# kakaobrain/hqtransformer

Hardware: AMD Instinct MI355X
Metric: images/sec (256x256 class-cond sampling) (higher is better)
Workload: dtype bf16

## Files before the change

### hqtransformer_amd/csrc/engine.hip

```cpp
#include "../../include/hqt.h"
#include "kernels.h"
#include "fast_kernels.h"
#include "split_kernels.h"
#include "persist.h"

#include <algorithm>
#include <cmath>
#include <cstdarg>
#include <cstdio>
#include <cstring>
#include <map>
#include <memory>
#include <mutex>
#include <string>
#include <vector>

static thread_local std::string g_err;
static int fail(int code, const char* fmt, ...) {
    char buf[1024];
    va_list ap;
    va_start(ap, fmt);
    vsnprintf(buf, sizeof(buf), fmt, ap);
    va_end(ap);
    g_err = buf;
// ... 84 lines not shown
    std::map<std::string, Tensor> w;
    std::vector<void*> owned;
    size_t workspace_bytes = 0;
    int64_t params[3] = {0, 0, 0};
    std::vector<BlockW> body, depth;
    Lin head_top, head_bot;
    int Tmax = 0;
    int max_prefix = 0;
    static constexpr int BODY_BUFS = 10;
    size_t body_bytes[BODY_BUFS] = {};
    int depth_rows = 0;
    int score_chunk = 0;
    int depth_cap() const { return std::max(cfg.max_batch, score_chunk); }
    static constexpr int DEPTH_BUFS = 4;
    size_t depth_bytes[DEPTH_BUFS] = {};
    float *x = nullptr, *xd = nullptr, *logits = nullptr;
    void *hbuf = nullptr, *qbuf = nullptr, *abuf = nullptr, *mbuf = nullptr;
    void *kcache = nullptr, *vcache = nullptr, *dk = nullptr, *dv = nullptr;
    bf16_t *xpk = nullptr, *xdpk = nullptr;
    float *parts = nullptr, *partsd = nullptr;
    int nparts = 0, npartsd = 0;
    float* fold_tmp = nullptr;
    bool tile_gemm = true;
    float* splitk = nullptr;
    size_t splitk_elems = 0;
    struct { const float* slabs; int S; int rows; const float* bias; } pend = {nullptr, 0, 0, nullptr};
    StepState* state = nullptr;
    RowKey* rows = nullptr;
    static constexpr int ROWS_RING = 4;
    RowKey* rows_pinned[ROWS_RING] = {nullptr, nullptr, nullptr, nullptr};
    hipEvent_t rows_ev[ROWS_RING] = {nullptr, nullptr, nullptr, nullptr};
    bool rows_busy[ROWS_RING] = {false, false, false, false};
    int rows_next = 0;
    RowSampler* row_set = nullptr;
    GuidePair* guide = nullptr;
    size_t guide_room() const { return (size_t)std::max(1, cfg.max_batch / 2); }
    unsigned char* keep_mask = nullptr;
    int* group_of_row = nullptr;
    int* row_pos = nullptr;
    struct Staged {
        std::vector<hqt_row_sampler> row_set;
        float* logprob = nullptr;
        std::vector<hqt_guide_pair> guide;
        std::vector<uint8_t> keep;
        int keep_B = 0, keep_n = 0;
        const int64_t* keep_codes[3] = {nullptr, nullptr, nullptr};
// ... 199 lines not shown
        }
    }
    if (c.s1_use_mid_block) {
        add(1, "encoder.mid.block_1", block_in, block_in, res);
        if (c.s1_use_attn) add(2, "encoder.mid.attn_1", block_in, block_in, res);
        add(1, "encoder.mid.block_2", block_in, block_in, res);
    }
    add(7, "encoder", block_in, c.s1_z_channels, res);
}

extern "C" int hqt_abi_version(void) { return HQT_ABI_VERSION; }
extern "C" const char* hqt_last_error(void) { return g_err.c_str(); }

static int alloc_workspace(hqt_handle* hp);

extern "C" int hqt_create(const hqt_config* cfg, int device, hqt_handle** out) {
    if (!cfg || !out) return fail(HQT_ERR_INVALID, "null argument");
    if (cfg->abi_version != HQT_ABI_VERSION) return fail(HQT_ERR_INVALID, "abi_version %d != %d", cfg->abi_version, HQT_ABI_VERSION);
    if (cfg->max_batch < 1) return fail(HQT_ERR_INVALID, "max_batch must be >= 1");
    DeviceGuard dg(device);
    if (!dg.ok) return fail(HQT_ERR_HIP, "hipSetDevice(%d) failed", device);
    std::unique_ptr<hqt_handle> h(new hqt_handle());
    h->tile_gemm = getenv("HQT_NO_TILE_GEMM") == nullptr;
    { const char* e = getenv("HQT_PERSIST"); h->persist_enabled = !(e && atoi(e) == 0); }
    h->single_key = getenv("HQT_NO_SINGLE_KEY") == nullptr;
    h->split_kslices = getenv("HQT_SPLIT_KSLICES_OFF") == nullptr;
    h->cfg = *cfg;
    h->layouts = (cfg->ar_layouts & HQT_LAYOUT_ALL) ? (cfg->ar_layouts & HQT_LAYOUT_ALL) : HQT_LAYOUT_ALL;
    h->device = device;
    const hqt_config& c = h->cfg;
    if (c.has_stage2) {
        if (c.embed_dim % c.n_heads || c.embed_dim % 16) return fail(HQT_ERR_INVALID, "embed_dim must be a multiple of n_heads and 16");
        const int hs = c.embed_dim / c.n_heads;
        if (hs % 8 || hs > 256 || (hs & (hs - 1))) return fail(HQT_ERR_INVALID, "head_dim %d unsupported (power of two in [8, 256])", hs);
        if (c.vocab_top != c.vocab_bot) return fail(HQT_ERR_INVALID, "vocab_top != vocab_bot");
        const bool bidir = c.depth_decoding == HQT_DEPTH_BIDIRECTIONAL;
        if (c.depth_decoding < 0 || c.depth_decoding > HQT_DEPTH_BIDIRECTIONAL || (c.depth_decoding && !bidir && c.code_levels != 3) || (bidir && c.code_levels == 3))
            return fail(HQT_ERR_INVALID, "depth_decoding %d: 0 'parallel-add', 1 'parallel', 2 'parallel-reduce', 3 'top2mid2bot' (three code levels only), "
                        "4 'bidirectional' (two code levels only)", c.depth_decoding);
        if (bidir && c.cond_type == HQT_COND_TEXT)
            return fail(HQT_ERR_INVALID, "depth_decoding 4 'bidirectional' with text conditioning is not built");
        if (c.vocab_top > HQT_MAX_V || c.vocab_top % 4) return fail(HQT_ERR_INVALID, "vocab size %d unsupported", c.vocab_top);
        if (c.cond_type == HQT_COND_CLASS && c.n_classes < 1) return fail(HQT_ERR_INVALID, "n_classes");
        if (c.max_steps < 1 || c.max_steps > c.ctx_len_img) return fail(HQT_ERR_INVALID, "max_steps must be in [1, ctx_len_img]");
    }
    if (c.has_stage1) {
// ... 600 lines not shown
    g.tune = h->policy;
    if (g.alpha == 0.0f) g.alpha = 1.0f;
    if (g.lda == 0) g.lda = l.K;
    if (split_planes) { g.Bw = l.w16h; g.Bw_lo = l.w16l; g.Bw_frag16 = l.wfrag16; g.Bw_up16 = l.wup16; }
}

struct SlotName {
    char s[64];
    SlotName(const char* tag, int rows) {
        static const bool by_rows = getenv("HQT_TIMING_BY_ROWS") != nullptr;
        snprintf(s, sizeof s, by_rows ? "%s@%d" : "%s", tag, rows);
    }
};

static int ar_linear(hqt_handle* h, const Mode& md, GemmArgs g, const Lin& l, int a_dt, int c_dt, hipStream_t st,
                     const char* tag, bool defer_residual = false, int* resid_nparts = nullptr) {
    lin_args(h, g, l, false);
    g.k_quarters = 1;
    const SlotName slot(tag, g.M);
    Timed t(h, slot.s, st);
    if (md.fast) {
        if (resid_nparts) *resid_nparts = g.N / 32;
        if ((g.ln_parts ? l.wpk_ln : l.wpk) && h->tile_gemm && tile_gemm_ok(g, a_dt, c_dt)) {
            const TilePlan tp = tile_gemm_plan(g);
            if (tp.geom >= 0 && (size_t)tp.S * 32 * g.a_packed_mb * g.N <= h->splitk_elems) {
                if (g.ln_parts) g.bias = l.bias_ln;
                HIPCHK(launch_tile_gemm(g, g.ln_parts ? l.wpk_ln : l.wpk, a_dt, c_dt, tp, h->splitk, st));
                if (tp.S > 1) {
                    count_variant(h, "variant:tile_gemm_%dx%d_splitk%d:%s", tp.bm, tp.bn, tp.S, slot.s);
                    t.next(SlotName("gemm_combine", g.M).s);
                    HIPCHK(launch_resid_combine(g, h->splitk, tp.S, st));
                } else count_variant(h, "variant:tile_gemm_%dx%d%s:%s", tp.bm, tp.bn, g.ln_parts ? "_dln" : "", slot.s);
                if (resid_nparts) *resid_nparts = tp.S > 1 ? 1 : g.N / tp.bn;
                return HQT_OK;
            }
        }
        if (g.ln_parts) {
            if (!l.wpk_ln || !stream_gemm_ok(g, a_dt, c_dt)) return fail(HQT_ERR_STATE, "deferred-LayerNorm GEMM without folded weights (%s)", tag);
            g.bias = l.bias_ln;
            HIPCHK(launch_stream_gemm(g, l.wpk_ln, a_dt, c_dt, 1, nullptr, st));
            count_variant(h, "variant:stream_gemm_dln:%s", tag);
            return HQT_OK;
        }
        if (l.wpk && stream_gemm_ok(g, a_dt, c_dt)) {
            int S = (defer_residual && g.store != STORE_RESID) ? stream_gemm_splitk(g) : 1;
            if ((size_t)S * 32 * g.a_packed_mb * g.N > h->splitk_elems) S = 1;
            HIPCHK(launch_stream_gemm(g, l.wpk, a_dt, c_dt, S, h->splitk, st));
            count_variant(h, "variant:stream_gemm:%s", tag);
            if (S > 1) h->pend = {h->splitk, S, 32 * g.a_packed_mb, l.b32};
            return HQT_OK;
        }
        g.Bw = l.w16;
        if (mfma_gemm_ok(g, a_dt, DT_BF16, c_dt)) {
            HIPCHK(launch_mfma_gemm(g, a_dt, DT_BF16, c_dt, st));
            count_variant(h, "variant:mfma_gemm:%s", tag);
// ... 1784 lines not shown
```

### hqtransformer_amd/csrc/fast_kernels.h

```cpp
#pragma once
#include "common.h"
#include "kernels.h"

hipError_t launch_f32_to_bf16(const float* src, bf16_t* dst, size_t n, hipStream_t st);
hipError_t launch_repack_conv(const float* src, float* dst, int O, int I, int taps, hipStream_t st, int Ipad = 0);

bool stream_gemm_supported(int N, int K);
hipError_t launch_pack_stream_weights(const float* w32, bf16_t* packed, int N, int K, hipStream_t st);
hipError_t launch_fold_layernorm(const float* w32, const float* gamma, const float* beta, const float* bias, float* wfold_tmp,
                                 bf16_t* packed, float* colsum, float* bias_out, int N, int K, hipStream_t st);
bool stream_gemm_ok(const GemmArgs& g, int a_dt, int c_dt);
hipError_t stream_gemm_configure();
int stream_gemm_splitk(const GemmArgs& g);
hipError_t launch_stream_gemm(const GemmArgs& g, const bf16_t* wpk, int a_dt, int c_dt, int S, float* slabs, hipStream_t st);

struct TilePlan { int geom; int bm, bn; int S; };
constexpr int TILE_CTR_MAX = 4096;
bool tile_gemm_ok(const GemmArgs& g, int a_dt, int c_dt);
TilePlan tile_gemm_plan(const GemmArgs& g);
hipError_t launch_tile_gemm(const GemmArgs& g, const bf16_t* wpk, int a_dt, int c_dt, const TilePlan& p, float* slabs, hipStream_t st);
hipError_t launch_resid_combine(const GemmArgs& g, const float* slabs, int S, hipStream_t st);
hipError_t tile_gemm_configure();

bool mfma_gemm_ok(const GemmArgs& g, int a_dt, int b_dt, int c_dt);
hipError_t launch_mfma_gemm(const GemmArgs& g, int a_dt, int b_dt, int c_dt, hipStream_t st);
bool conv_halo_ok(const GemmArgs& g, int c_dt);
bool conv_halo_stats_ok(int N, int groups);
int conv_halo_tiles_per_image(const GemmArgs& g);
hipError_t mfma_gemm_configure();
```

### hqtransformer_amd/csrc/tile_gemm.hip

```cpp
#include "fast_kernels.h"
#include "gemm_generic.h"
#include <algorithm>
#include <type_traits>

typedef __attribute__((ext_vector_type(8))) __bf16 bf16x8;
typedef __attribute__((ext_vector_type(16))) float f32x16;
typedef __attribute__((ext_vector_type(4))) float f32x4;

enum { TS_QKV = 0, TS_PACKED = 1, TS_RESID = 2, TS_ROWS = 3, TS_SLAB = 4,
       TS_FUSED = 5 };
typedef __attribute__((ext_vector_type(4))) unsigned u32x4;
#ifndef HQT_TILE_STAGGER
#define HQT_TILE_STAGGER 1
#endif

template <int WGM_, int WGN_, int MBW_, int NT_, int KU_, int NSTAGE_, int NLOAD_ = 0>
struct TileGeom {
    static constexpr int WGM = WGM_, WGN = WGN_, MBW = MBW_, NT = NT_, KU = KU_, NSTAGE = NSTAGE_, NLOAD = NLOAD_;
    static constexpr int NC = WGM * WGN;
    static constexpr int NW = NC + NLOAD;
    static constexpr int NDMA = NLOAD ? NLOAD : NC;
    static constexpr int BM = 32 * MBW * WGM, BN = 32 * NT * WGN;
    static constexpr int ACH = BM / 32, WCH = BN / 32;
    static constexpr int CPS = ACH + WCH;
// ... 30 lines not shown

__device__ __forceinline__ void tile_of(int b, int total, int S, int TM, int TN, int& z, int& tm, int& tn) {
    int t;
    if (S > 1 && (8 % S) == 0) {
        const int xcd = b & 7, G = 8 / S, xg = xcd / S;
        z = xcd - xg * S;
        const int q = total / G, r = total - q * G;
        t = (xg < r ? xg * (q + 1) : r * (q + 1) + (xg - r) * q) + (b >> 3);
    } else {
        z = b / total;
        const int id = b - z * total;
        const int q = total >> 3, r = total & 7, xcd = id & 7;
        t = (xcd < r ? xcd * (q + 1) : r * (q + 1) + (xcd - r) * q) + (id >> 3);
    }
    const int nb = TM <= 12 ? 1 : (TM + 7) >> 3;
    const int GM = (TM + nb - 1) / nb;
    const int per_group = GM * TN;
    const int group = t / per_group, in_group = t - group * per_group;
    const int first = group * GM, rows = min(TM - first, GM);
    tn = in_group / rows;
    tm = first + in_group - tn * rows;
}

template <class G, int STORE, bool DLN, typename TC, int ACT = ACT_NONE>
__global__ __launch_bounds__(G::NW * 64, (G::NW / 4) * G::WG_PER_CU) void tile_gemm_kernel(GemmArgs g, const char* __restrict__ wpk,
                                                                                              float* __restrict__ slabs, int TM, int TN) {
#if defined(__HIP_DEVICE_COMPILE__)
    constexpr int WGM = G::WGM, MBW = G::MBW, NT = G::NT, KU = G::KU, NSTAGE = G::NSTAGE, NW = G::NW, NC = G::NC, NLOAD = G::NLOAD, NDMA = G::NDMA;
    constexpr int BM = G::BM, BN = G::BN, ACH = G::ACH, CPS = G::CPS, CPW = G::CPW, STAGE = G::STAGE_BYTES;
    extern __shared__ __attribute__((aligned(1024))) char lds[];
    float* const meanrstd = reinterpret_cast<float*>(lds + G::RING_BYTES);
    float* const colb = meanrstd + 2 * BM;
    float* const scratch = colb + 2 * BN;
#ifdef HQT_TILE_STAMPS
    long long stamp[8];
    stamp[5] = stamp[6] = stamp[7] = 0;
    stamp[0] = wall_clock64(); stamp[1] = clock64();
#endif
    const int wave = __builtin_amdgcn_readfirstlane(threadIdx.x >> 6), lane = threadIdx.x & 63;
    const int wm = wave % WGM, wn = wave / WGM;
    const bool loader = NLOAD > 0 && wave >= NC;
    const int dw = NLOAD > 0 ? max(wave - NC, 0) : wave;
    const int total = TM * TN;
    const int S = gridDim.x / total;
    int z, tile_m, tile_n;
    tile_of(blockIdx.x, total, S, TM, TN, z, tile_m, tile_n);
    const int m0 = tile_m * BM, n0 = tile_n * BN;
    const int MB = g.a_packed_mb, KS = g.K >> 4, NTILES = g.N >> 5;
    const int ks_lo = (int)(((long long)KS * z) / S), ks_hi = (int)(((long long)KS * (z + 1)) / S);
    const int KT = (ks_hi - ks_lo) / KU;

    const auto rsA = __builtin_amdgcn_make_buffer_rsrc(const_cast<void*>(g.A), 0, 0xFFFFFFFF, 0x00020000);
// ... 11 lines not shown
        } else {
            const int fw = f - NA, ku = fw / G::WCH, r = fw - ku * G::WCH;
            off[i] = (unsigned)(((size_t)min(tile_n * G::WCH + r, NTILES - 1) * KS + ks_lo + ku) * 1024);
            dstoff[i] = (ku * CPS + ACH + r) * 1024;
        }
    }
    const unsigned stepA = (unsigned)KU * MB * 1024, stepW = KU * 1024;
    const int lane16 = lane * 16;
    auto issue = [&](int slot) {
#pragma unroll
        for (int i = 0; i < CPW; ++i) {
            char* dst = lds + slot * STAGE + dstoff[i];
            if (i < NA / NDMA) {
                __builtin_amdgcn_raw_ptr_buffer_load_lds(rsA, (__attribute__((address_space(3))) void*)dst, 16, lane16, off[i], 0, 0);
                off[i] += stepA;
            } else {
                __builtin_amdgcn_raw_ptr_buffer_load_lds(rsW, (__attribute__((address_space(3))) void*)dst, 16, lane16, off[i], 0, 0);
                off[i] += stepW;
            }
        }
    };

    f32x16 acc[NT][MBW];
#pragma unroll
    for (int j = 0; j < NT; ++j)
#pragma unroll
        for (int i = 0; i < MBW; ++i)
#pragma unroll
            for (int r = 0; r < 16; ++r) acc[j][i][r] = 0.0f;

    float bias_r = 0.0f, cs_r = 0.0f;
    const int pc = min((int)threadIdx.x, BN - 1);
    if (STORE != TS_SLAB) {
        const float* zsrc = reinterpret_cast<const float*>(g.A);
        const int n = min(n0 + pc, g.N - 1);
        bias_r = *(g.bias ? g.bias + n : zsrc);
        cs_r = *(DLN ? g.ln_colsum + n : zsrc);
    }
    constexpr int NPL = 6;
    float2 pv[NPL];
    const int pr = threadIdx.x % BM, pgi = threadIdx.x / BM;
    if (DLN && !loader) {
        const float2* base = reinterpret_cast<const float2*>(g.ln_parts) + min(m0 + pr, MB * 32 - 1);
#pragma unroll
        for (int i = 0; i < NPL; ++i) pv[i] = base[(size_t)min(pgi + i * G::GR, g.ln_nparts - 1) * (MB * 32)];
    }
    __builtin_amdgcn_sched_barrier(0);
    if (NLOAD == 0 || loader) {
#pragma unroll
        for (int s = 0; s < NSTAGE; ++s) issue(s);
    }
    __builtin_amdgcn_sched_barrier(0);
// ... 10 lines not shown
            const float2* base = reinterpret_cast<const float2*>(g.ln_parts) + min(m0 + pr, MB * 32 - 1);
            for (int p0 = pgi + NPL * G::GR; p0 < g.ln_nparts; p0 += G::GR) { const float2 v = base[(size_t)p0 * (MB * 32)]; sm += v.x; sq += v.y; }
        }
        if (!loader) {
            scratch[2 * threadIdx.x] = sm;
            scratch[2 * threadIdx.x + 1] = sq;
        }
        asm volatile("s_waitcnt lgkmcnt(0)" ::: "memory");
        __builtin_amdgcn_s_barrier();
        __builtin_amdgcn_sched_barrier(0);
        if (threadIdx.x < BM) {
            float a = 0.0f, b = 0.0f;
#pragma unroll
            for (int k = 0; k < G::GR; ++k) { a += scratch[2 * (k * BM + threadIdx.x)]; b += scratch[2 * (k * BM + threadIdx.x) + 1]; }
            const float mean = a / (float)g.K;
            const float var = fmaxf(b / (float)g.K - mean * mean, 0.0f);
            meanrstd[2 * threadIdx.x] = mean;
            meanrstd[2 * threadIdx.x + 1] = 1.0f / sqrtf(var + g.ln_eps);
        }
    }
    const int qkv_row_dev = (STORE == TS_QKV && g.row_offset_dev) ? *g.row_offset_dev : 0;

    bf16x8 af[2][MBW], wf[2][NT];
    auto read_frags = [&](auto set_tag, int slot, int ku) {
        constexpr int SET = decltype(set_tag)::value;
        const char* st = lds + slot * STAGE + ku * (CPS * 1024) + lane * 16;
#pragma unroll
        for (int j = 0; j < NT; ++j) wf[SET][j] = *reinterpret_cast<const bf16x8*>(st + (ACH + wn * NT + j) * 1024);
#pragma unroll
        for (int i = 0; i < MBW; ++i) af[SET][i] = *reinterpret_cast<const bf16x8*>(st + (wm * MBW + i) * 1024);
    };
    auto multiply = [&](auto set_tag) {
        constexpr int SET = decltype(set_tag)::value;
#pragma unroll
        for (int j = 0; j < NT; ++j)
#pragma unroll
            for (int i = 0; i < MBW; ++i) acc[j][i] = __builtin_amdgcn_mfma_f32_32x32x16_bf16(wf[SET][j], af[SET][i], acc[j][i], 0, 0, 0);
    };
    auto wait_stage = [&](int younger) {
        constexpr int MAXY = (63 / CPW) < (NSTAGE - 1) ? (63 / CPW) : (NSTAGE - 1);
        if (MAXY >= 5 && younger >= 5) wait_vmcnt<MAXY >= 5 ? CPW * 5 : 0>();
        else if (MAXY >= 4 && younger >= 4) wait_vmcnt<MAXY >= 4 ? CPW * 4 : 0>();
        else if (MAXY >= 3 && younger >= 3) wait_vmcnt<MAXY >= 3 ? CPW * 3 : 0>();
        else if (MAXY >= 2 && younger >= 2) wait_vmcnt<MAXY >= 2 ? CPW * 2 : 0>();
        else if (MAXY >= 1 && younger >= 1) wait_vmcnt<CPW>();
        else wait_vmcnt<0>();
    };
    const bool early = NW < 8 || wave < NW / 2 || HQT_TILE_STAGGER == 0;
    if (NLOAD > 0 && loader) {
        wait_stage(NSTAGE - 1);
        __builtin_amdgcn_s_barrier();
        int slot = 0;
        for (int kt = 0; kt < KT - 1; ++kt) {
            wait_stage(min(NSTAGE - 2, KT - 2 - kt));
            __builtin_amdgcn_s_barrier();
            if (kt + NSTAGE < KT) issue(slot);
            slot = slot + 1 == NSTAGE ? 0 : slot + 1;
        }
        return;
    }
    if (NLOAD == 0) wait_stage(NSTAGE - 1);
    __builtin_amdgcn_s_barrier();
    __builtin_amdgcn_sched_barrier(0);
#ifdef HQT_TILE_STAMPS
    stamp[2] = clock64();
#endif
    __builtin_amdgcn_s_waitcnt(0xC07F);
    read_frags(std::integral_constant<int, 0>{}, 0, 0);
    int rd = 0;
    auto stage = [&](auto par_tag, auto last_tag, int kt) {
        constexpr int P = decltype(par_tag)::value;
        constexpr bool LAST = decltype(last_tag)::value;
#pragma unroll
        for (int ku = 0; ku < KU; ++ku) {
            const bool cur1 = ((P + ku) & 1) != 0;
            if (ku < KU - 1) {
                if (cur1) { read_frags(std::integral_constant<int, 0>{}, rd, ku + 1); __builtin_amdgcn_sched_barrier(0); multiply(std::integral_constant<int, 1>{}); }
                else { read_frags(std::integral_constant<int, 1>{}, rd, ku + 1); __builtin_amdgcn_sched_barrier(0); multiply(std::integral_constant<int, 0>{}); }
                __builtin_amdgcn_sched_barrier(0);
            } else {
                const int nxt = rd + 1 == NSTAGE ? 0 : rd + 1;
                if (!LAST) {
                    if (NLOAD == 0) wait_stage(min(NSTAGE - 2, KT - 2 - kt));
                    asm volatile("s_waitcnt lgkmcnt(0)" ::: "memory");
                    __builtin_amdgcn_s_barrier();
                    __builtin_amdgcn_sched_barrier(0);
                    if (NLOAD == 0 && early && kt + NSTAGE < KT) issue(rd);
                    if (cur1) read_frags(std::integral_constant<int, 0>{}, nxt, 0);
                    else read_frags(std::integral_constant<int, 1>{}, nxt, 0);
                    __builtin_amdgcn_sched_barrier(0);
                }
                if (cur1) multiply(std::integral_constant<int, 1>{});
                else multiply(std::integral_constant<int, 0>{});
                __builtin_amdgcn_sched_barrier(0);
                if (NLOAD == 0 && !LAST && !early && kt + NSTAGE < KT) issue(rd);
                __builtin_amdgcn_sched_barrier(0);
                rd = nxt;
            }
        }
    };
    constexpr std::integral_constant<int, 0> P0{};
    constexpr std::integral_constant<int, 1> P1{};
    constexpr std::false_type MORE{};
    constexpr std::true_type FINAL{};
    if (KU % 2 == 0) {
        for (int kt = 0; kt < KT - 1; ++kt) stage(P0, MORE, kt);
        stage(P0, FINAL, KT - 1);
    } else {
        int kt = 0;
        for (; kt + 2 < KT; kt += 2) { stage(P0, MORE, kt); stage(P1, MORE, kt + 1); }
        if (kt + 2 == KT) { stage(P0, MORE, kt); stage(P1, FINAL, kt + 1); }
        else stage(P0, FINAL, kt);
    }

#ifdef HQT_TILE_STAMPS
    __builtin_amdgcn_sched_barrier(0);
    asm volatile("s_nop 15\n\ts_nop 15" ::: "memory");
    stamp[3] = clock64();
    __builtin_amdgcn_sched_barrier(0);
#endif
    const int c = lane & 31, h = lane >> 5;
    const int Mc = g.c_packed_mb * 32;
    constexpr int WCOLS = 32 * NT, PITCH = WCOLS + 4;
    float* const stg = reinterpret_cast<float*>(lds) + wave * (32 * PITCH);
    static_assert(NC * 32 * PITCH * 4 <= G::RING_BYTES, "staging patches fit the ring");
    float mean[MBW], rstd[MBW];
#pragma unroll
    for (int i = 0; i < MBW; ++i) {
        mean[i] = DLN ? meanrstd[2 * ((wm * MBW + i) * 32 + c)] : 0.0f;
        rstd[i] = DLN ? meanrstd[2 * ((wm * MBW + i) * 32 + c) + 1] : 1.0f;
    }
    const int qkv_part_local = STORE == TS_QKV ? n0 / max(g.qkv_D, 1) : 0;
    const int qkv_part = qkv_part_local + g.qkv_first;
    bf16_t* const qkv_base = reinterpret_cast<bf16_t*>(qkv_part == 0 ? g.C : (qkv_part == 1 ? g.C2 : g.C3));
    bf16_t* const qkv_vcopy = (STORE == TS_QKV && qkv_part == 2) ? g.qkv_v_pk : nullptr;
    const auto rs_qkv = __builtin_amdgcn_make_buffer_rsrc(qkv_base, 0, 0xFFFFFFFF, 0x00020000);
    float* const slab_out = STORE == TS_SLAB ? slabs + (size_t)z * (MB * 32) * g.N : nullptr;
    const auto rs_slab = __builtin_amdgcn_make_buffer_rsrc(STORE == TS_FUSED ? slabs : nullptr, 0, 0xFFFFFFFF, 0x00020000);
    const unsigned slab_stride = (unsigned)((size_t)(MB * 32) * g.N * 4);
    float rs[MBW], rq[MBW];
#pragma unroll
    for (int i = 0; i < MBW; ++i) rs[i] = rq[i] = 0.0f;
    const int wcol0 = n0 + wn * WCOLS;
    if (STORE != TS_PACKED) __syncthreads();
    static_assert(STORE != TS_FUSED || (!DLN && G::NLOAD >= 0), "TS_FUSED: plain residual producers");
#ifdef HQT_TILE_STAMPS
    __builtin_amdgcn_sched_barrier(0);
    stamp[5] = clock64();
    __builtin_amdgcn_sched_barrier(0);
#endif
    auto run_epilogue = [&](auto mode_c, auto from_slabs_c) {
    constexpr int MODE = decltype(mode_c)::value;
    constexpr bool FROM_SLABS = decltype(from_slabs_c)::value;
#pragma unroll
    for (int i = 0; i < MBW; ++i) {
        const int mrow0 = m0 + (wm * MBW + i) * 32;
#pragma unroll
        for (int j = 0; j < NT; ++j)
#pragma unroll
            for (int q4 = 0; q4 < 4; ++q4) {
                if (FROM_SLABS) continue;
                const int cl = j * 32 + 8 * q4 + 4 * h;
                float v[4];
                if (MODE == TS_SLAB) {
#pragma unroll
                    for (int e = 0; e < 4; ++e) v[e] = acc[j][i][4 * q4 + e];
                } else {
                    const f32x4 b4 = *reinterpret_cast<const f32x4*>(colb + wn * WCOLS + cl);
                    const f32x4 cs4 = *reinterpret_cast<const f32x4*>(colb + BN + wn * WCOLS + cl);
#pragma unroll
                    for (int e = 0; e < 4; ++e) {
                        float t = acc[j][i][4 * q4 + e];
                        if (DLN) t = rstd[i] * (t - mean[i] * cs4[e]);
                        v[e] = t * g.alpha + b4[e];
                    }
                }
                if (MODE == TS_PACKED) {
#pragma unroll
                    for (int e = 0; e < 4; ++e) v[e] = tile_act<ACT>(v[e]);
                    if (mrow0 + c < g.M) st4<bf16_t>(reinterpret_cast<bf16_t*>(g.C) + packed_off(mrow0 + c, wcol0 + cl, g.c_packed_mb), v);
                    continue;
                }
                if (MODE == TS_ROWS) {
#pragma unroll
                    for (int e = 0; e < 4; ++e) v[e] = tile_act<ACT>(v[e]);
                }
                if (qkv_vcopy && mrow0 + c < g.M) st4<bf16_t>(qkv_vcopy + packed_off(mrow0 + c, wcol0 + cl - qkv_part_local * g.qkv_D, g.c_packed_mb), v);
                *reinterpret_cast<f32x4*>(stg + c * PITCH + cl) = f32x4{v[0], v[1], v[2], v[3]};
            }
        if (MODE == TS_PACKED) continue;
        __builtin_amdgcn_fence(__ATOMIC_ACQ_REL, "wavefront");
        __builtin_amdgcn_wave_barrier();
        if (MODE == TS_SLAB || MODE == TS_RESID || (MODE == TS_ROWS && sizeof(TC) == 4)) {
            constexpr int LPR = WCOLS / 4, RPP = 64 / LPR, NP = 32 / RPP;
            const int cg = (lane % LPR) * 4, r0 = lane / LPR;
            float* const out = MODE == TS_SLAB ? slab_out : reinterpret_cast<float*>(g.C);
            const int ldo = MODE == TS_SLAB ? g.N : g.ldc;
            f32x4 x0[NP];
            if (MODE == TS_RESID) {
#pragma unroll
                for (int p = 0; p < NP; ++p) {
                    const int m = min(mrow0 + p * RPP + r0, g.M - 1);
                    x0[p] = *reinterpret_cast<const f32x4*>(out + (size_t)m * ldo + wcol0 + cg);
                }
            }
            if (FROM_SLABS) {
                const f32x4 b4 = *reinterpret_cast<const f32x4*>(colb + wn * WCOLS + cg);
                constexpr int HP = NP / 2;
#pragma unroll
                for (int hp = 0; hp < 2; ++hp) {
                    u32x4 pz[8][HP];
// ... 168 lines not shown
        pk.y = (unsigned)hb[2] | ((unsigned)hb[3] << 16);
        *reinterpret_cast<uint2*>(xpk + packed_off(m, n4, pk_mb)) = pk;
    }
#pragma unroll
    for (int off = 32; off > 0; off >>= 1) { rs += __shfl_xor(rs, off, 64); rq += __shfl_xor(rq, off, 64); }
    constexpr int NWV = NT / 64;
    if ((threadIdx.x & 63) == 0) { red[threadIdx.x >> 6] = rs; red[NWV + (threadIdx.x >> 6)] = rq; }
    __syncthreads();
    if (threadIdx.x == 0) {
        float a = 0.0f, b = 0.0f;
#pragma unroll
        for (int w = 0; w < NWV; ++w) { a += red[w]; b += red[NWV + w]; }
        parts[2 * m] = a;
        parts[2 * m + 1] = b;
    }
}

typedef TileGeom<2, 2, 2, 2, 2, 3> Tile128;
typedef TileGeom<2, 2, 1, 2, 2, 3> Tile64;
typedef TileGeom<2, 4, 1, 1, 4, 3> Tile64W8;
typedef TileGeom<2, 2, 2, 2, 2, 4, 4> Tile128PC;
typedef TileGeom<2, 2, 1, 1, 4, 3> Tile64x64;

template <class G, int STORE, bool DLN, typename TC, int ACT = ACT_NONE>
static hipError_t launch_tile_t(const GemmArgs& g, const bf16_t* wpk, int S, float* slabs, hipStream_t st) {
    const int TM = (g.M + G::BM - 1) / G::BM, TN = (g.N + G::BN - 1) / G::BN;
    tile_gemm_kernel<G, STORE, DLN, TC, ACT><<<TM * TN * S, G::NW * 64, G::LDS_BYTES, st>>>(g, reinterpret_cast<const char*>(wpk), slabs, TM, TN);
    return hipGetLastError();
}
template <class G, bool DLN>
static hipError_t launch_tile_packed(const GemmArgs& g, const bf16_t* wpk, hipStream_t st) {
    switch (g.act) {
    case ACT_NONE: return launch_tile_t<G, TS_PACKED, DLN, bf16_t, ACT_NONE>(g, wpk, 1, nullptr, st);
    case ACT_GELU_ERF: return launch_tile_t<G, TS_PACKED, DLN, bf16_t, ACT_GELU_ERF>(g, wpk, 1, nullptr, st);
    case ACT_GELU_SIGMOID: return launch_tile_t<G, TS_PACKED, DLN, bf16_t, ACT_GELU_SIGMOID>(g, wpk, 1, nullptr, st);
    }
    return hipErrorInvalidValue;
}

template <class G>
static hipError_t launch_tile_g(const GemmArgs& g, const bf16_t* wpk, int c_dt, int S, float* slabs, hipStream_t st) {
    const bool dln = g.ln_parts != nullptr;
    if (S > 1) return launch_tile_t<G, TS_SLAB, false, float>(g, wpk, S, slabs, st);
    switch (g.store) {
    case STORE_QKV: return dln ? launch_tile_t<G, TS_QKV, true, bf16_t>(g, wpk, 1, nullptr, st) : launch_tile_t<G, TS_QKV, false, bf16_t>(g, wpk, 1, nullptr, st);
    case STORE_PACKED: return dln ? launch_tile_packed<G, true>(g, wpk, st) : launch_tile_packed<G, false>(g, wpk, st);
    case STORE_RESID: return launch_tile_t<G, TS_RESID, false, float>(g, wpk, 1, nullptr, st);
    case STORE_ROWS:
        if (c_dt == DT_F32) return dln ? launch_tile_t<G, TS_ROWS, true, float>(g, wpk, 1, nullptr, st) : launch_tile_t<G, TS_ROWS, false, float>(g, wpk, 1, nullptr, st);
        return dln ? launch_tile_t<G, TS_ROWS, true, bf16_t>(g, wpk, 1, nullptr, st) : launch_tile_t<G, TS_ROWS, false, bf16_t>(g, wpk, 1, nullptr, st);
    }
    return hipErrorInvalidValue;
}

bool tile_gemm_ok(const GemmArgs& g, int a_dt, int c_dt) {
    if (!(g.a_packed_mb >= 16 && a_dt == DT_BF16 && !g.conv_taps && g.batch <= 1 && g.M >= 512)) return false;
    if (g.N % 128 != 0 || g.K % 32 != 0 || g.K < 256 || g.ldc % 8 != 0 || g.resid) return false;
    if (g.act != ACT_NONE && g.store != STORE_PACKED) return false;
    if (g.store == STORE_QKV) return c_dt == DT_BF16 && g.qkv_D % 128 == 0 && g.rows_per_group > 0;
    if (g.store == STORE_PACKED) return c_dt == DT_BF16 && g.c_packed_mb > 0;
    if (g.store == STORE_RESID) return c_dt == DT_F32 && g.c_packed_mb > 0 && !g.ln_parts && g.resid_pk && g.resid_parts && g.N == g.ldc && (g.K >= 3072 || g.M >= 640);
    if (g.store == STORE_ROWS) return g.rows_per_group == 0 && g.act == ACT_NONE;
    return false;
}

TilePlan tile_gemm_plan(const GemmArgs& g) {
    constexpr int max_s = 8;
    TilePlan p{0, Tile128::BM, Tile128::BN, 1};
    const int KS = g.K / 16, tiles = ((g.M + p.bm - 1) / p.bm) * (g.N / p.bn);
    if (g.store == STORE_RESID && g.K < 3072 && ((g.M + 63) / 64) * (g.N / 64) <= 256 && KS % Tile64x64::KU == 0 && KS / Tile64x64::KU >= 2 * Tile64x64::NSTAGE)
        return TilePlan{3, 64, 64, 1};
    if (g.store != STORE_RESID && tiles >= 160 && tiles <= 256 && KS % Tile128PC::KU == 0 && KS / Tile128PC::KU >= 2 * Tile128PC::NSTAGE)
        return TilePlan{4, Tile128PC::BM, Tile128PC::BN, 1};
    if (g.store != STORE_RESID && tiles < 256 && KS / Tile64::KU >= Tile64::NSTAGE) {
        const int t64 = ((g.M + Tile64::BM - 1) / Tile64::BM) * (g.N / Tile64::BN);
        if (t64 <= 512 && KS % Tile64W8::KU == 0 && KS / Tile64W8::KU >= 2 * Tile64W8::NSTAGE) return TilePlan{2, Tile64::BM, Tile64::BN, 1};
        return TilePlan{1, Tile64::BM, Tile64::BN, 1};
    }
    if (g.store == STORE_RESID && g.K < 3072 && tiles < 256 && KS % Tile64W8::KU == 0 && KS / Tile64W8::KU >= 2 * Tile64W8::NSTAGE)
        return TilePlan{2, Tile64::BM, Tile64::BN, 1};
    if (g.store == STORE_RESID && g.K >= 3072 && tiles >= 160 && tiles <= 256 && KS % Tile128PC::KU == 0 && KS / Tile128PC::KU >= 2 * Tile128PC::NSTAGE)
        return TilePlan{4, Tile128PC::BM, Tile128PC::BN, 1};
    if (g.store == STORE_RESID && g.K >= 3072 && tiles < 256) {
        const int t64 = ((g.M + Tile64::BM - 1) / Tile64::BM) * (g.N / Tile64::BN);
        if (((t64 >= 176 && t64 <= 208) || (t64 >= 448 && t64 <= 512)) && KS % Tile64W8::KU == 0 && KS / Tile64W8::KU >= 2 * Tile64W8::NSTAGE)
            return TilePlan{2, Tile64::BM, Tile64::BN, 1};
        if ((tiles * 4 <= 256 || tiles % 64 == 0) && KS % (Tile128::KU * 4) == 0 && KS / 4 / Tile128::KU >= 2 * Tile128::NSTAGE) {
            p.S = 4;
            if (tiles * 4 <= 256 && KS / 4 / Tile128PC::KU >= 2 * Tile128PC::NSTAGE) p.geom = 4;
            return p;
        }
        for (int S : {8, 6, 4, 3, 2})
            if (S <= max_s && tiles * S <= 576 && KS % (Tile128::KU * S) == 0 && KS / S / Tile128::KU >= 2 * Tile128::NSTAGE) { p.S = S; break; }
    }
    return p;
}

hipError_t launch_tile_gemm(const GemmArgs& g, const bf16_t* wpk, int a_dt, int c_dt, const TilePlan& p, float* slabs, hipStream_t st) {
    (void)a_dt;
    const GemmArgs& gg = g;
    if (p.geom == 0) return launch_tile_g<Tile128>(gg, wpk, c_dt, p.S, slabs, st);
    if (p.geom == 1) return launch_tile_g<Tile64>(gg, wpk, c_dt, p.S, slabs, st);
    if (p.geom == 2) return launch_tile_g<Tile64W8>(gg, wpk, c_dt, p.S, slabs, st);
    if (p.geom == 3) return launch_tile_g<Tile64x64>(gg, wpk, c_dt, p.S, slabs, st);
    if (p.geom == 4) return launch_tile_g<Tile128PC>(gg, wpk, c_dt, p.S, slabs, st);
    return hipErrorInvalidValue;
}

hipError_t launch_resid_combine(const GemmArgs& g, const float* slabs, int S, hipStream_t st) {
    float* x = reinterpret_cast<float*>(g.C);
    const int rows = g.a_packed_mb * 32;
    switch (S) {
#define COMBINE(S_) case S_:                                                                                                                          \
        if (g.N == 1536) resid_combine_kernel<S_, 384><<<g.M, 384, 0, st>>>(x, slabs, g.bias, g.resid_pk, g.resid_parts, g.M, g.N, rows, g.c_packed_mb);     \
        else resid_combine_kernel<S_, 256><<<g.M, 256, 0, st>>>(x, slabs, g.bias, g.resid_pk, g.resid_parts, g.M, g.N, rows, g.c_packed_mb);                 \
        break;
    COMBINE(2) COMBINE(3) COMBINE(4) COMBINE(6) COMBINE(8)
#undef COMBINE
    default: return hipErrorInvalidValue;
    }
    return hipGetLastError();
}

template <class G, int STORE, bool DLN, typename TC, int ACT = ACT_NONE>
static hipError_t configure_one() {
    void (*kernel)(GemmArgs, const char*, float*, int, int) = tile_gemm_kernel<G, STORE, DLN, TC, ACT>;
    return hipFuncSetAttribute(reinterpret_cast<const void*>(kernel), hipFuncAttributeMaxDynamicSharedMemorySize, G::LDS_BYTES);
}
template <class G>
static hipError_t configure_g() {
    hipError_t e;
#define CFG(STORE, DLN, TC)                      \
    e = configure_one<G, STORE, DLN, TC>();      \
    if (e != hipSuccess) return e;
    CFG(TS_QKV, true, bf16_t) CFG(TS_QKV, false, bf16_t) CFG(TS_PACKED, true, bf16_t) CFG(TS_PACKED, false, bf16_t)
    CFG(TS_RESID, false, float) CFG(TS_ROWS, true, float) CFG(TS_ROWS, false, float) CFG(TS_ROWS, true, bf16_t) CFG(TS_ROWS, false, bf16_t)
    CFG(TS_SLAB, false, float)
#undef CFG
    for (hipError_t e2 : {configure_one<G, TS_PACKED, true, bf16_t, ACT_GELU_ERF>(), configure_one<G, TS_PACKED, false, bf16_t, ACT_GELU_ERF>(),
                          configure_one<G, TS_PACKED, true, bf16_t, ACT_GELU_SIGMOID>(), configure_one<G, TS_PACKED, false, bf16_t, ACT_GELU_SIGMOID>()})
        if (e2 != hipSuccess) return e2;
    return hipSuccess;
}
hipError_t tile_gemm_configure() {
    hipError_t e = configure_g<Tile128>();
    if (e == hipSuccess) e = configure_g<Tile64>();
    if (e == hipSuccess) e = configure_g<Tile64W8>();
    if (e == hipSuccess) e = configure_g<Tile64x64>();
    if (e == hipSuccess) e = configure_g<Tile128PC>();
    return e;
}
```

Measured before the change: 1692.

## Add 16x16x32 MFMA variant of tile GEMM, default for large-M Tile128

Adds a template parameter to the tile GEMM kernel that selects a 16x16x32 bf16 MFMA path instead of 32x32 MFMA. This changes the LDS fragment reads, the accumulator layout and the epilogue row/column mapping to match. By default it is used only for geometry 0 (Tile128) when M is at least 2048, and an env var can force it on or off. The aim is higher MFMA throughput and better instruction scheduling on MI355X for large GEMMs. In exchange it doubles the number of kernel instantiations and increases register pressure from the extra fragment arrays.

```diff
diff --git a/hqtransformer_amd/csrc/engine.hip b/hqtransformer_amd/csrc/engine.hip
--- a/hqtransformer_amd/csrc/engine.hip
+++ b/hqtransformer_amd/csrc/engine.hip
@@ -130,6 +130,7 @@
     int nparts = 0, npartsd = 0;
     float* fold_tmp = nullptr;
     bool tile_gemm = true;
+    int tile_mfma = 0;
     float* splitk = nullptr;
     size_t splitk_elems = 0;
     struct { const float* slabs; int S; int rows; const float* bias; } pend = {nullptr, 0, 0, nullptr};
@@ -375,6 +376,7 @@
     if (!dg.ok) return fail(HQT_ERR_HIP, "hipSetDevice(%d) failed", device);
     std::unique_ptr<hqt_handle> h(new hqt_handle());
     h->tile_gemm = getenv("HQT_NO_TILE_GEMM") == nullptr;
+    { const char* e = getenv("HQT_TILE_MFMA"); const int v = e ? atoi(e) : 0; h->tile_mfma = v == 16 || v == 32 ? v : 0; }
     { const char* e = getenv("HQT_PERSIST"); h->persist_enabled = !(e && atoi(e) == 0); }
     h->single_key = getenv("HQT_NO_SINGLE_KEY") == nullptr;
     h->split_kslices = getenv("HQT_SPLIT_KSLICES_OFF") == nullptr;
@@ -1021,15 +1023,15 @@
     if (md.fast) {
         if (resid_nparts) *resid_nparts = g.N / 32;
         if ((g.ln_parts ? l.wpk_ln : l.wpk) && h->tile_gemm && tile_gemm_ok(g, a_dt, c_dt)) {
-            const TilePlan tp = tile_gemm_plan(g);
+            const TilePlan tp = tile_gemm_plan(g, h->tile_mfma);
             if (tp.geom >= 0 && (size_t)tp.S * 32 * g.a_packed_mb * g.N <= h->splitk_elems) {
                 if (g.ln_parts) g.bias = l.bias_ln;
                 HIPCHK(launch_tile_gemm(g, g.ln_parts ? l.wpk_ln : l.wpk, a_dt, c_dt, tp, h->splitk, st));
                 if (tp.S > 1) {
-                    count_variant(h, "variant:tile_gemm_%dx%d_splitk%d:%s", tp.bm, tp.bn, tp.S, slot.s);
+                    count_variant(h, "variant:tile_gemm_%dx%d%s_splitk%d:%s", tp.bm, tp.bn, tp.mf == 16 ? "_mfma16" : "", tp.S, slot.s);
                     t.next(SlotName("gemm_combine", g.M).s);
                     HIPCHK(launch_resid_combine(g, h->splitk, tp.S, st));
-                } else count_variant(h, "variant:tile_gemm_%dx%d%s:%s", tp.bm, tp.bn, g.ln_parts ? "_dln" : "", slot.s);
+                } else count_variant(h, "variant:tile_gemm_%dx%d%s%s:%s", tp.bm, tp.bn, tp.mf == 16 ? "_mfma16" : "", g.ln_parts ? "_dln" : "", slot.s);
                 if (resid_nparts) *resid_nparts = tp.S > 1 ? 1 : g.N / tp.bn;
                 return HQT_OK;
             }
diff --git a/hqtransformer_amd/csrc/fast_kernels.h b/hqtransformer_amd/csrc/fast_kernels.h
--- a/hqtransformer_amd/csrc/fast_kernels.h
+++ b/hqtransformer_amd/csrc/fast_kernels.h
@@ -14,10 +14,10 @@
 int stream_gemm_splitk(const GemmArgs& g);
 hipError_t launch_stream_gemm(const GemmArgs& g, const bf16_t* wpk, int a_dt, int c_dt, int S, float* slabs, hipStream_t st);
 
-struct TilePlan { int geom; int bm, bn; int S; };
+struct TilePlan { int geom; int bm, bn; int S; int mf; };
 constexpr int TILE_CTR_MAX = 4096;
 bool tile_gemm_ok(const GemmArgs& g, int a_dt, int c_dt);
-TilePlan tile_gemm_plan(const GemmArgs& g);
+TilePlan tile_gemm_plan(const GemmArgs& g, int mfma = 0);
 hipError_t launch_tile_gemm(const GemmArgs& g, const bf16_t* wpk, int a_dt, int c_dt, const TilePlan& p, float* slabs, hipStream_t st);
 hipError_t launch_resid_combine(const GemmArgs& g, const float* slabs, int S, hipStream_t st);
 hipError_t tile_gemm_configure();
diff --git a/hqtransformer_amd/csrc/tile_gemm.hip b/hqtransformer_amd/csrc/tile_gemm.hip
--- a/hqtransformer_amd/csrc/tile_gemm.hip
+++ b/hqtransformer_amd/csrc/tile_gemm.hip
@@ -76,12 +76,15 @@
     tm = first + in_group - tn * rows;
 }
 
-template <class G, int STORE, bool DLN, typename TC, int ACT = ACT_NONE>
+template <class G, int STORE, bool DLN, typename TC, int ACT = ACT_NONE, int MF = 32>
 __global__ __launch_bounds__(G::NW * 64, (G::NW / 4) * G::WG_PER_CU) void tile_gemm_kernel(GemmArgs g, const char* __restrict__ wpk,
                                                                                               float* __restrict__ slabs, int TM, int TN) {
 #if defined(__HIP_DEVICE_COMPILE__)
     constexpr int WGM = G::WGM, MBW = G::MBW, NT = G::NT, KU = G::KU, NSTAGE = G::NSTAGE, NW = G::NW, NC = G::NC, NLOAD = G::NLOAD, NDMA = G::NDMA;
     constexpr int BM = G::BM, BN = G::BN, ACH = G::ACH, CPS = G::CPS, CPW = G::CPW, STAGE = G::STAGE_BYTES;
+    constexpr bool MF16 = MF == 16;
+    static_assert(MF == 32 || (MF == 16 && KU % 2 == 0), "16x16x32: whole pairs of k-steps per stage");
+    constexpr int KSTEPS = MF16 ? KU / 2 : KU;
     extern __shared__ __attribute__((aligned(1024))) char lds[];
     float* const meanrstd = reinterpret_cast<float*>(lds + G::RING_BYTES);
     float* const colb = meanrstd + 2 * BM;
@@ -139,12 +142,16 @@
     };
 
     f32x16 acc[NT][MBW];
+    f32x4 acc16[NT][MBW][4];
 #pragma unroll
     for (int j = 0; j < NT; ++j)
 #pragma unroll
         for (int i = 0; i < MBW; ++i)
 #pragma unroll
-            for (int r = 0; r < 16; ++r) acc[j][i][r] = 0.0f;
+            for (int r = 0; r < 16; ++r) {
+                if (MF16) acc16[j][i][r >> 2][r & 3] = 0.0f;
+                else acc[j][i][r] = 0.0f;
+            }
 
     float bias_r = 0.0f, cs_r = 0.0f;
     const int pc = min((int)threadIdx.x, BN - 1);
@@ -201,8 +208,22 @@
     const int qkv_row_dev = (STORE == TS_QKV && g.row_offset_dev) ? *g.row_offset_dev : 0;
 
     bf16x8 af[2][MBW], wf[2][NT];
+    bf16x8 af16[2][MBW][2], wf16[2][NT][2];
+    const int lane_off16 = (lane >> 5) * (CPS * 1024) + (((lane >> 4) & 1) * 32 + (lane & 15)) * 16;
     auto read_frags = [&](auto set_tag, int slot, int ku) {
         constexpr int SET = decltype(set_tag)::value;
+        if (MF16) {
+            const char* st = lds + slot * STAGE + ku * (2 * CPS * 1024) + lane_off16;
+#pragma unroll
+            for (int j = 0; j < NT; ++j)
+#pragma unroll
+                for (int rh = 0; rh < 2; ++rh) wf16[SET][j][rh] = *reinterpret_cast<const bf16x8*>(st + (ACH + wn * NT + j) * 1024 + rh * 256);
+#pragma unroll
+            for (int i = 0; i < MBW; ++i)
+#pragma unroll
+                for (int rh = 0; rh < 2; ++rh) af16[SET][i][rh] = *reinterpret_cast<const bf16x8*>(st + (wm * MBW + i) * 1024 + rh * 256);
+            return;
+        }
         const char* st = lds + slot * STAGE + ku * (CPS * 1024) + lane * 16;
 #pragma unroll
         for (int j = 0; j < NT; ++j) wf[SET][j] = *reinterpret_cast<const bf16x8*>(st + (ACH + wn * NT + j) * 1024);
@@ -211,6 +232,16 @@
     };
     auto multiply = [&](auto set_tag) {
         constexpr int SET = decltype(set_tag)::value;
+        if (MF16) {
+#pragma unroll
+            for (int j = 0; j < NT; ++j)
+#pragma unroll
+                for (int i = 0; i < MBW; ++i)
+#pragma unroll
+                    for (int q = 0; q < 4; ++q)
+                        acc16[j][i][q] = __builtin_amdgcn_mfma_f32_16x16x32_bf16(wf16[SET][j][q & 1], af16[SET][i][q >> 1], acc16[j][i][q], 0, 0, 0);
+            return;
+        }
 #pragma unroll
         for (int j = 0; j < NT; ++j)
 #pragma unroll
@@ -251,9 +282,9 @@
         constexpr int P = decltype(par_tag)::value;
         constexpr bool LAST = decltype(last_tag)::value;
 #pragma unroll
-        for (int ku = 0; ku < KU; ++ku) {
+        for (int ku = 0; ku < KSTEPS; ++ku) {
             const bool cur1 = ((P + ku) & 1) != 0;
-            if (ku < KU - 1) {
+            if (ku < KSTEPS - 1) {
                 if (cur1) { read_frags(std::integral_constant<int, 0>{}, rd, ku + 1); __builtin_amdgcn_sched_barrier(0); multiply(std::integral_constant<int, 1>{}); }
                 else { read_frags(std::integral_constant<int, 1>{}, rd, ku + 1); __builtin_amdgcn_sched_barrier(0); multiply(std::integral_constant<int, 0>{}); }
                 __builtin_amdgcn_sched_barrier(0);
@@ -282,14 +313,28 @@
     constexpr std::integral_constant<int, 1> P1{};
     constexpr std::false_type MORE{};
     constexpr std::true_type FINAL{};
-    if (KU % 2 == 0) {
+    if (KSTEPS % 2 == 0) {
         for (int kt = 0; kt < KT - 1; ++kt) stage(P0, MORE, kt);
         stage(P0, FINAL, KT - 1);
     } else {
         int kt = 0;
         for (; kt + 2 < KT; kt += 2) { stage(P0, MORE, kt); stage(P1, MORE, kt + 1); }
-        if (kt + 2 == KT) { stage(P0, MORE, kt); stage(P1, FINAL, kt + 1); }
-        else stage(P0, FINAL, kt);
+        if (kt + 2 == KT) {
+            stage(P0, MORE, kt);
+            if (MF16) {
+#pragma unroll
+                for (int j = 0; j < (NT); ++j) { wf16[0][j][0] = wf16[1][j][0]; wf16[0][j][1] = wf16[1][j][1]; }
+#pragma unroll
+                for (int i = 0; i < (MBW); ++i) { af16[0][i][0] = af16[1][i][0]; af16[0][i][1] = af16[1][i][1]; }
+            } else {
+#pragma unroll
+                for (int j = 0; j < (NT); ++j) wf[0][j] = wf[1][j];
+#pragma unroll
+                for (int i = 0; i < (MBW); ++i) af[0][i] = af[1][i];
+            }
+            ++kt;
+        }
+        stage(P0, FINAL, kt);
     }
 
 #ifdef HQT_TILE_STAMPS
@@ -303,12 +348,16 @@
     constexpr int WCOLS = 32 * NT, PITCH = WCOLS + 4;
     float* const stg = reinterpret_cast<float*>(lds) + wave * (32 * PITCH);
     static_assert(NC * 32 * PITCH * 4 <= G::RING_BYTES, "staging patches fit the ring");
-    float mean[MBW], rstd[MBW];
-#pragma unroll
-    for (int i = 0; i < MBW; ++i) {
-        mean[i] = DLN ? meanrstd[2 * ((wm * MBW + i) * 32 + c)] : 0.0f;
-        rstd[i] = DLN ? meanrstd[2 * ((wm * MBW + i) * 32 + c) + 1] : 1.0f;
-    }
+    const int c16 = lane & 15, h16 = lane >> 4;
+    float mean[MBW][2], rstd[MBW][2];
+#pragma unroll
+    for (int i = 0; i < MBW; ++i)
+#pragma unroll
+        for (int mh = 0; mh < 2; ++mh) {
+            const int r = (wm * MBW + i) * 32 + (MF16 ? 16 * mh + c16 : c);
+            mean[i][mh] = DLN ? meanrstd[2 * r] : 0.0f;
+            rstd[i][mh] = DLN ? meanrstd[2 * r + 1] : 1.0f;
+        }
     const int qkv_part_local = STORE == TS_QKV ? n0 / max(g.qkv_D, 1) : 0;
     const int qkv_part = qkv_part_local + g.qkv_first;
     bf16_t* const qkv_base = reinterpret_cast<bf16_t*>(qkv_part == 0 ? g.C : (qkv_part == 1 ? g.C2 : g.C3));
@@ -339,33 +388,38 @@
 #pragma unroll
             for (int q4 = 0; q4 < 4; ++q4) {
                 if (FROM_SLABS) continue;
-                const int cl = j * 32 + 8 * q4 + 4 * h;
+                const int cl = MF16 ? j * 32 + 16 * (q4 & 1) + 4 * h16 : j * 32 + 8 * q4 + 4 * h;
+                const int rl = MF16 ? 16 * (q4 >> 1) + c16 : c;
+                const int mh = MF16 ? q4 >> 1 : 0;
+                float a4[4];
+#pragma unroll
+                for (int e = 0; e < 4; ++e) a4[e] = MF16 ? acc16[j][i][q4][e] : acc[j][i][4 * q4 + e];
                 float v[4];
                 if (MODE == TS_SLAB) {
 #pragma unroll
-                    for (int e = 0; e < 4; ++e) v[e] = acc[j][i][4 * q4 + e];
+                    for (int e = 0; e < 4; ++e) v[e] = a4[e];
                 } else {
                     const f32x4 b4 = *reinterpret_cast<const f32x4*>(colb + wn * WCOLS + cl);
                     const f32x4 cs4 = *reinterpret_cast<const f32x4*>(colb + BN + wn * WCOLS + cl);
 #pragma unroll
                     for (int e = 0; e < 4; ++e) {
-                        float t = acc[j][i][4 * q4 + e];
-                        if (DLN) t = rstd[i] * (t - mean[i] * cs4[e]);
+                        float t = a4[e];
+                        if (DLN) t = rstd[i][mh] * (t - mean[i][mh] * cs4[e]);
                         v[e] = t * g.alpha + b4[e];
                     }
                 }
                 if (MODE == TS_PACKED) {
 #pragma unroll
                     for (int e = 0; e < 4; ++e) v[e] = tile_act<ACT>(v[e]);
-                    if (mrow0 + c < g.M) st4<bf16_t>(reinterpret_cast<bf16_t*>(g.C) + packed_off(mrow0 + c, wcol0 + cl, g.c_packed_mb), v);
+                    if (mrow0 + rl < g.M) st4<bf16_t>(reinterpret_cast<bf16_t*>(g.C) + packed_off(mrow0 + rl, wcol0 + cl, g.c_packed_mb), v);
                     continue;
                 }
                 if (MODE == TS_ROWS) {
 #pragma unroll
                     for (int e = 0; e < 4; ++e) v[e] = tile_act<ACT>(v[e]);
                 }
-                if (qkv_vcopy && mrow0 + c < g.M) st4<bf16_t>(qkv_vcopy + packed_off(mrow0 + c, wcol0 + cl - qkv_part_local * g.qkv_D, g.c_packed_mb), v);
-                *reinterpret_cast<f32x4*>(stg + c * PITCH + cl) = f32x4{v[0], v[1], v[2], v[3]};
+                if (qkv_vcopy && mrow0 + rl < g.M) st4<bf16_t>(qkv_vcopy + packed_off(mrow0 + rl, wcol0 + cl - qkv_part_local * g.qkv_D, g.c_packed_mb), v);
+                *reinterpret_cast<f32x4*>(stg + rl * PITCH + cl) = f32x4{v[0], v[1], v[2], v[3]};
             }
         if (MODE == TS_PACKED) continue;
         __builtin_amdgcn_fence(__ATOMIC_ACQ_REL, "wavefront");
@@ -580,33 +634,34 @@
 typedef TileGeom<2, 2, 2, 2, 2, 4, 4> Tile128PC;
 typedef TileGeom<2, 2, 1, 1, 4, 3> Tile64x64;
 
-template <class G, int STORE, bool DLN, typename TC, int ACT = ACT_NONE>
+template <class G, int STORE, bool DLN, typename TC, int ACT = ACT_NONE, int MF = 32>
 static hipError_t launch_tile_t(const GemmArgs& g, const bf16_t* wpk, int S, float* slabs, hipStream_t st) {
     const int TM = (g.M + G::BM - 1) / G::BM, TN = (g.N + G::BN - 1) / G::BN;
-    tile_gemm_kernel<G, STORE, DLN, TC, ACT><<<TM * TN * S, G::NW * 64, G::LDS_BYTES, st>>>(g, reinterpret_cast<const char*>(wpk), slabs, TM, TN);
+    tile_gemm_kernel<G, STORE, DLN, TC, ACT, MF><<<TM * TN * S, G::NW * 64, G::LDS_BYTES, st>>>(g, reinterpret_cast<const char*>(wpk), slabs, TM, TN);
     return hipGetLastError();
 }
-template <class G, bool DLN>
+template <class G, bool DLN, int MF>
 static hipError_t launch_tile_packed(const GemmArgs& g, const bf16_t* wpk, hipStream_t st) {
     switch (g.act) {
-    case ACT_NONE: return launch_tile_t<G, TS_PACKED, DLN, bf16_t, ACT_NONE>(g, wpk, 1, nullptr, st);
-    case ACT_GELU_ERF: return launch_tile_t<G, TS_PACKED, DLN, bf16_t, ACT_GELU_ERF>(g, wpk, 1, nullptr, st);
-    case ACT_GELU_SIGMOID: return launch_tile_t<G, TS_PACKED, DLN, bf16_t, ACT_GELU_SIGMOID>(g, wpk, 1, nullptr, st);
+    case ACT_NONE: return launch_tile_t<G, TS_PACKED, DLN, bf16_t, ACT_NONE, MF>(g, wpk, 1, nullptr, st);
+    case ACT_GELU_ERF: return launch_tile_t<G, TS_PACKED, DLN, bf16_t, ACT_GELU_ERF, MF>(g, wpk, 1, nullptr, st);
+    case ACT_GELU_SIGMOID: return launch_tile_t<G, TS_PACKED, DLN, bf16_t, ACT_GELU_SIGMOID, MF>(g, wpk, 1, nullptr, st);
     }
     return hipErrorInvalidValue;
 }
 
-template <class G>
+template <class G, int MF>
 static hipError_t launch_tile_g(const GemmArgs& g, const bf16_t* wpk, int c_dt, int S, float* slabs, hipStream_t st) {
     const bool dln = g.ln_parts != nullptr;
-    if (S > 1) return launch_tile_t<G, TS_SLAB, false, float>(g, wpk, S, slabs, st);
+    constexpr int A0 = ACT_NONE;
+    if (S > 1) return launch_tile_t<G, TS_SLAB, false, float, A0, MF>(g, wpk, S, slabs, st);
     switch (g.store) {
-    case STORE_QKV: return dln ? launch_tile_t<G, TS_QKV, true, bf16_t>(g, wpk, 1, nullptr, st) : launch_tile_t<G, TS_QKV, false, bf16_t>(g, wpk, 1, nullptr, st);
-    case STORE_PACKED: return dln ? launch_tile_packed<G, true>(g, wpk, st) : launch_tile_packed<G, false>(g, wpk, st);
-    case STORE_RESID: return launch_tile_t<G, TS_RESID, false, float>(g, wpk, 1, nullptr, st);
+    case STORE_QKV: return dln ? launch_tile_t<G, TS_QKV, true, bf16_t, A0, MF>(g, wpk, 1, nullptr, st) : launch_tile_t<G, TS_QKV, false, bf16_t, A0, MF>(g, wpk, 1, nullptr, st);
+    case STORE_PACKED: return dln ? launch_tile_packed<G, true, MF>(g, wpk, st) : launch_tile_packed<G, false, MF>(g, wpk, st);
+    case STORE_RESID: return launch_tile_t<G, TS_RESID, false, float, A0, MF>(g, wpk, 1, nullptr, st);
     case STORE_ROWS:
-        if (c_dt == DT_F32) return dln ? launch_tile_t<G, TS_ROWS, true, float>(g, wpk, 1, nullptr, st) : launch_tile_t<G, TS_ROWS, false, float>(g, wpk, 1, nullptr, st);
-        return dln ? launch_tile_t<G, TS_ROWS, true, bf16_t>(g, wpk, 1, nullptr, st) : launch_tile_t<G, TS_ROWS, false, bf16_t>(g, wpk, 1, nullptr, st);
+        if (c_dt == DT_F32) return dln ? launch_tile_t<G, TS_ROWS, true, float, A0, MF>(g, wpk, 1, nullptr, st) : launch_tile_t<G, TS_ROWS, false, float, A0, MF>(g, wpk, 1, nullptr, st);
+        return dln ? launch_tile_t<G, TS_ROWS, true, bf16_t, A0, MF>(g, wpk, 1, nullptr, st) : launch_tile_t<G, TS_ROWS, false, bf16_t, A0, MF>(g, wpk, 1, nullptr, st);
     }
     return hipErrorInvalidValue;
 }
@@ -622,7 +677,7 @@
     return false;
 }
 
-TilePlan tile_gemm_plan(const GemmArgs& g) {
+static TilePlan plan_geometry(const GemmArgs& g) {
     constexpr int max_s = 8;
     TilePlan p{0, Tile128::BM, Tile128::BN, 1};
     const int KS = g.K / 16, tiles = ((g.M + p.bm - 1) / p.bm) * (g.N / p.bn);
@@ -654,15 +709,30 @@
     return p;
 }
 
+constexpr unsigned TILE_MFMA16_GEOMS = 1u << 0;
+constexpr int TILE_MFMA16_MIN_ROWS = 2048;
+constexpr unsigned TILE_MFMA16_BUILT = 0xFu;
+static_assert((TILE_MFMA16_GEOMS & ~TILE_MFMA16_BUILT) == 0, "a geometry adopted with 16x16x32 is built with it");
+
+TilePlan tile_gemm_plan(const GemmArgs& g, int mfma) {
+    TilePlan p = plan_geometry(g);
+    const unsigned take = mfma == 16 ? TILE_MFMA16_BUILT : (mfma == 32 || g.M < TILE_MFMA16_MIN_ROWS ? 0u : TILE_MFMA16_GEOMS);
+    p.mf = p.geom >= 0 && ((take >> p.geom) & 1u) ? 16 : 32;
+    return p;
+}
+
+template <int MF>
+static hipError_t launch_tile_mf(const GemmArgs& g, const bf16_t* wpk, int c_dt, const TilePlan& p, float* slabs, hipStream_t st) {
+    if (p.geom == 0) return launch_tile_g<Tile128, MF>(g, wpk, c_dt, p.S, slabs, st);
+    if (p.geom == 1) return launch_tile_g<Tile64, MF>(g, wpk, c_dt, p.S, slabs, st);
+    if (p.geom == 2) return launch_tile_g<Tile64W8, MF>(g, wpk, c_dt, p.S, slabs, st);
+    if (p.geom == 3) return launch_tile_g<Tile64x64, MF>(g, wpk, c_dt, p.S, slabs, st);
+    if (p.geom == 4 && MF == 32) return launch_tile_g<Tile128PC, 32>(g, wpk, c_dt, p.S, slabs, st);
+    return hipErrorInvalidValue;
+}
 hipError_t launch_tile_gemm(const GemmArgs& g, const bf16_t* wpk, int a_dt, int c_dt, const TilePlan& p, float* slabs, hipStream_t st) {
     (void)a_dt;
-    const GemmArgs& gg = g;
-    if (p.geom == 0) return launch_tile_g<Tile128>(gg, wpk, c_dt, p.S, slabs, st);
-    if (p.geom == 1) return launch_tile_g<Tile64>(gg, wpk, c_dt, p.S, slabs, st);
-    if (p.geom == 2) return launch_tile_g<Tile64W8>(gg, wpk, c_dt, p.S, slabs, st);
-    if (p.geom == 3) return launch_tile_g<Tile64x64>(gg, wpk, c_dt, p.S, slabs, st);
-    if (p.geom == 4) return launch_tile_g<Tile128PC>(gg, wpk, c_dt, p.S, slabs, st);
-    return hipErrorInvalidValue;
+    return p.mf == 16 ? launch_tile_mf<16>(g, wpk, c_dt, p, slabs, st) : launch_tile_mf<32>(g, wpk, c_dt, p, slabs, st);
 }
 
 hipError_t launch_resid_combine(const GemmArgs& g, const float* slabs, int S, hipStream_t st) {
@@ -680,31 +750,36 @@
     return hipGetLastError();
 }
 
-template <class G, int STORE, bool DLN, typename TC, int ACT = ACT_NONE>
+template <class G, int MF, int STORE, bool DLN, typename TC, int ACT = ACT_NONE>
 static hipError_t configure_one() {
-    void (*kernel)(GemmArgs, const char*, float*, int, int) = tile_gemm_kernel<G, STORE, DLN, TC, ACT>;
+    void (*kernel)(GemmArgs, const char*, float*, int, int) = tile_gemm_kernel<G, STORE, DLN, TC, ACT, MF>;
     return hipFuncSetAttribute(reinterpret_cast<const void*>(kernel), hipFuncAttributeMaxDynamicSharedMemorySize, G::LDS_BYTES);
 }
-template <class G>
+template <class G, int MF>
 static hipError_t configure_g() {
     hipError_t e;
 #define CFG(STORE, DLN, TC)                      \
-    e = configure_one<G, STORE, DLN, TC>();      \
+    e = configure_one<G, MF, STORE, DLN, TC>();  \
     if (e != hipSuccess) return e;
     CFG(TS_QKV, true, bf16_t) CFG(TS_QKV, false, bf16_t) CFG(TS_PACKED, true, bf16_t) CFG(TS_PACKED, false, bf16_t)
     CFG(TS_RESID, false, float) CFG(TS_ROWS, true, float) CFG(TS_ROWS, false, float) CFG(TS_ROWS, true, bf16_t) CFG(TS_ROWS, false, bf16_t)
     CFG(TS_SLAB, false, float)
 #undef CFG
-    for (hipError_t e2 : {configure_one<G, TS_PACKED, true, bf16_t, ACT_GELU_ERF>(), configure_one<G, TS_PACKED, false, bf16_t, ACT_GELU_ERF>(),
-                          configure_one<G, TS_PACKED, true, bf16_t, ACT_GELU_SIGMOID>(), configure_one<G, TS_PACKED, false, bf16_t, ACT_GELU_SIGMOID>()})
+    for (hipError_t e2 : {configure_one<G, MF, TS_PACKED, true, bf16_t, ACT_GELU_ERF>(), configure_one<G, MF, TS_PACKED, false, bf16_t, ACT_GELU_ERF>(),
+                          configure_one<G, MF, TS_PACKED, true, bf16_t, ACT_GELU_SIGMOID>(), configure_one<G, MF, TS_PACKED, false, bf16_t, ACT_GELU_SIGMOID>()})
         if (e2 != hipSuccess) return e2;
     return hipSuccess;
 }
+template <int MF>
+static hipError_t configure_mf() {
+    hipError_t e = configure_g<Tile128, MF>();
+    if (e == hipSuccess) e = configure_g<Tile64, MF>();
+    if (e == hipSuccess) e = configure_g<Tile64W8, MF>();
+    if (e == hipSuccess) e = configure_g<Tile64x64, MF>();
+    if (e == hipSuccess && MF == 32) e = configure_g<Tile128PC, 32>();
+    return e;
+}
 hipError_t tile_gemm_configure() {
-    hipError_t e = configure_g<Tile128>();
-    if (e == hipSuccess) e = configure_g<Tile64>();
-    if (e == hipSuccess) e = configure_g<Tile64W8>();
-    if (e == hipSuccess) e = configure_g<Tile64x64>();
-    if (e == hipSuccess) e = configure_g<Tile128PC>();
-    return e;
-}
+    const hipError_t e = configure_mf<32>();
+    return e == hipSuccess ? configure_mf<16>() : e;
+}
```

Result: no change. 1700, median of 6 (+0.5%).
